# TGoldC/Motion-Planning-for-Autonomous-Driving-with-MPC

Hardware: AMD Instinct MI355X
Metric: MPC steps/sec (N=30, nx=6 nu=2) at batch=4096 (higher is better)
Workload: dtype f64; 1 GPU; N=30 nx=6 nu=2 bicycle lane-following, batch=4096/GPU, tol 1e-8; mode=converged, gpu=AMD Radeon Graphics

## Files before the change

### motion-planning-for-autonomous-driving-with-mpc_amd/csrc/mpc_host_common.h

```cpp
#pragma once
#include <cmath>
#include <cstddef>
#include <cstdint>
#include <cstdio>
#include <string>
#include <vector>

#include "../../include/mpcgpu.h"
#include "mpc_stage_math.h"

namespace mpc {

constexpr double BOUND_RELAX = 1e-8;

struct HostProblem {
    mpc_problem_desc desc{};
    std::vector<double> LB, UB;
    int has_fl = 0, has_fu = 0, has_ol = 0, has_ou = 0;
    double fl = 0, fu = 0, ol = 0, ou = 0;
    double ol_raw = 0;
    double fl_raw = 0;
    int fric_literal = 0;
    int n_mult = 0, n_z = 0;
    uint32_t lo_mask = 0, hi_mask = 0, dense_mask = 0xFFFFu;
    bool bounds_set = false;
    int NZ() const { return desc.nx + 2; }
    size_t n_w() const { return (size_t)2 * desc.N + (size_t)desc.nx * (desc.N + 1); }
    size_t n_g() const { return (size_t)1 + (size_t)desc.nx * (desc.N + 1) + (size_t)9 * (desc.N + 1); }
};

inline void apply_fric_literal(HostProblem& hp, int literal) {
    hp.fric_literal = literal ? 1 : 0;
    if (hp.bounds_set) hp.has_fl = std::isfinite(hp.fl_raw) && (hp.fl_raw > 0.0 || hp.fric_literal);
}
inline double relax_lo(double lo) { return std::isfinite(lo) ? lo - BOUND_RELAX * std::fmax(1.0, std::fabs(lo)) : -INFINITY; }
inline double relax_hi(double hi) { return std::isfinite(hi) ? hi + BOUND_RELAX * std::fmax(1.0, std::fabs(hi)) : INFINITY; }

inline int validate_desc(const mpc_problem_desc& d, std::string& err) {
    char buf[256];
    if (d.N < 1 || d.N > 127) { snprintf(buf, sizeof buf, "N=%d outside [1,127]", d.N); err = buf; return MPC_ERR_INVALID; }
    if (d.nx != 5 && d.nx != 6) { snprintf(buf, sizeof buf, "nx=%d (supported: 5, 6)", d.nx); err = buf; return MPC_ERR_INVALID; }
    if (d.nu != 2) { err = "nu must be 2"; return MPC_ERR_INVALID; }
    if (d.formulation != MPC_FORM_CASADI_EULER) { err = "unsupported formulation"; return MPC_ERR_INVALID; }
    if (!(d.dt > 0) || !(d.wheelbase > 0) || !(d.friction_div != 0) || !(d.tol > 0)) { err = "dt, wheelbase, tol must be > 0"; return MPC_ERR_INVALID; }
    if (d.obst_mult < 1 || d.max_iter < 1 || d.fixed_iters < 0) { err = "obst_mult>=1, max_iter>=1, fixed_iters>=0 required"; return MPC_ERR_INVALID; }
    if (d.max_iter > 1024 || d.fixed_iters > 1024) { err = "max_iter / fixed_iters above 1024 (the convergence-poll table)"; return MPC_ERR_INVALID; }
    return MPC_OK;
}

inline void default_bounds(const mpc_problem_desc& d, std::vector<double>& lbx, std::vector<double>& ubx,
                           std::vector<double>& lbg, std::vector<double>& ubg) {
    const int N = d.N, nx = d.nx;
    lbx.clear(); ubx.clear(); lbg.clear(); ubg.clear();
    for (int k = 0; k < N; ++k) { lbx.push_back(-0.4); ubx.push_back(0.4); lbx.push_back(-INFINITY); ubx.push_back(11.5); }
    for (int k = 0; k <= N; ++k) {
        const double lo[6] = {-INFINITY, -INFINITY, -1.066, 0.0, -INFINITY, -INFINITY};
        const double hi[6] = {INFINITY, INFINITY, 1.066, 50.8, INFINITY, INFINITY};
        for (int i = 0; i < nx; ++i) { lbx.push_back(lo[i]); ubx.push_back(hi[i]); }
    }
    lbg.push_back(0.0); ubg.push_back(11.5);
    for (int i = 0; i < nx * (N + 1); ++i) { lbg.push_back(0.0); ubg.push_back(0.0); }
    for (int i = 0; i < 9 * (N + 1); ++i) { lbg.push_back(1.2000000000000002); ubg.push_back(INFINITY); }
}

inline int set_bound_rows(HostProblem& hp, const double* lbx, const double* ubx, const double* lbg, const double* ubg, std::string& err) {
    const mpc_problem_desc& d = hp.desc;
    const int N = d.N, nx = d.nx, NZ = nx + 2;
    std::vector<double> dlbx, dubx, dlbg, dubg;
    if (!lbx && !ubx && !lbg && !ubg) {
        default_bounds(d, dlbx, dubx, dlbg, dubg);
        lbx = dlbx.data(); ubx = dubx.data(); lbg = dlbg.data(); ubg = dubg.data();
    } else if (!lbx || !ubx || !lbg || !ubg) {
        err = "lbx, ubx, lbg, ubg must be all given or all NULL";
        return MPC_ERR_INVALID;
    }
    char buf[256];
    hp.LB.assign((size_t)(N + 1) * NZ, -INFINITY);
    hp.UB.assign((size_t)(N + 1) * NZ, INFINITY);
    int nb = 0;
    for (int k = 0; k <= N; ++k)
        for (int i = 0; i < NZ; ++i) {
            if (i < 2 && k == N) continue;
            const size_t src = (i < 2) ? (size_t)2 * k + i : (size_t)2 * N + (size_t)nx * k + (i - 2);
            const double lo = lbx[src], hi = ubx[src];
            if (std::isnan(lo) || std::isnan(hi) || lo > hi) { snprintf(buf, sizeof buf, "lbx/ubx[%zu]: invalid pair", src); err = buf; return MPC_ERR_BOUNDS; }
            if (lo == hi) { snprintf(buf, sizeof buf, "lbx == ubx at %zu: fixed variables are not supported", src); err = buf; return MPC_ERR_BOUNDS; }
            hp.LB[(size_t)k * NZ + i] = relax_lo(lo);
            hp.UB[(size_t)k * NZ + i] = relax_hi(hi);
            if (!(k == 0 && i == 1)) nb += (int)std::isfinite(lo) + (int)std::isfinite(hi);
        }
    const double flo = lbg[0], fhi = ubg[0];
    if (std::isnan(flo) || std::isnan(fhi) || !(flo < fhi)) { err = "friction row needs lbg[0] < ubg[0]"; return MPC_ERR_BOUNDS; }
    for (int i = 0; i < nx * (N + 1); ++i)
        if (!(lbg[1 + i] == 0.0 && ubg[1 + i] == 0.0)) { snprintf(buf, sizeof buf, "g row %d must be an equality with lbg = ubg = 0", 1 + i); err = buf; return MPC_ERR_BOUNDS; }
    const size_t o0 = (size_t)1 + (size_t)nx * (N + 1);
    const double olo = lbg[o0], ohi = ubg[o0];
    for (int i = 0; i < 9 * (N + 1); ++i)
        if (!(lbg[o0 + i] == olo && ubg[o0 + i] == ohi)) { err = "obstacle rows must share one [lbg, ubg] pair"; return MPC_ERR_BOUNDS; }
    if (std::isnan(olo) || std::isnan(ohi) || !(olo < ohi)) { err = "obstacle rows need lbg < ubg"; return MPC_ERR_BOUNDS; }
    hp.fl_raw = flo;
    hp.has_fl = std::isfinite(flo) && (flo > 0.0 || hp.fric_literal);
    hp.has_fu = std::isfinite(fhi);
    hp.fl = relax_lo(flo); hp.fu = relax_hi(fhi);
    hp.has_ol = std::isfinite(olo); hp.has_ou = std::isfinite(ohi);
    hp.ol = relax_lo(olo); hp.ou = relax_hi(ohi);
    hp.ol_raw = olo;
    const int m = d.obst_mult;
    hp.n_mult = nx * (N + 1) + 3 * m * (N + 1);
    hp.n_z = nb + 3 * m * (N + 1) * (hp.has_ol + hp.has_ou);
    hp.bounds_set = true;
    return MPC_OK;
}
inline int set_bounds(HostProblem& hp, const double* lbx, const double* ubx, const double* lbg, const double* ubg, std::string& err) {
    const int rc = set_bound_rows(hp, lbx, ubx, lbg, ubg, err);
    hp.lo_mask = hp.hi_mask = 0;
    hp.dense_mask = 0xFFFFu;
    for (size_t q = 0; q < hp.LB.size(); ++q) {
        const int i = (int)(q % (size_t)hp.NZ()), k = (int)(q / (size_t)hp.NZ());
        if (hp.LB[q] > -1e300) hp.lo_mask |= 1u << i;
        if (hp.UB[q] < 1e300) hp.hi_mask |= 1u << i;
        if (!(i < 2 && k == hp.desc.N)) {
            if (!(hp.LB[q] > -1e300)) hp.dense_mask &= ~(1u << i);
            if (!(hp.UB[q] < 1e300)) hp.dense_mask &= ~(0x100u << i);
        }
    }
    return rc;
}

struct WsLayout {
    size_t Z, ZL, ZU, SO, NUO, ZLO, ZUO, LAM, REF, DZ, PK, KK, BLK, ROLL, SC, FILT, OBST;
    size_t MZ, MZL, MZU, MSO, MNUO, MZLO, MZUO, MLAM, MREF;
    size_t MBLK, MPK, MDZ;
    size_t rows, irows;
    size_t tile_elems, itile_elems, ntiles;
    size_t total, itotal;
    size_t elem(size_t row0, size_t row, size_t b) const { return (b >> 6) * tile_elems + mpc_prow((uint32_t)(row0 + row)) + (b & 63) * 2; }
    size_t ielem(size_t row, size_t b) const { return (b >> 6) * itile_elems + mpc_prow((uint32_t)row) + (b & 63) * 2; }
};

inline WsLayout ws_layout(int N, int nx, size_t Bp, bool mailbox = true) {
    const size_t NS = (size_t)nx * (nx + 1) / 2, S = N + 1;
    auto ev = [](size_t r) { return (r + 1) & ~(size_t)1; };
    const size_t NZ = ev(nx + 2), XS = ev(nx), NBLK = ev((nx + 5) + 10 + 2 * nx), NPK = ev(NS + nx), NKK = 2 * nx + 2;
    WsLayout w{};
    size_t off = 0;
    auto take = [&](size_t rows) { const size_t o = off; off += ev(rows); return o; };
    w.Z = take(S * NZ); w.ZL = take(S * NZ); w.ZU = take(S * NZ);
    w.SO = take(S * 4); w.NUO = take(S * 4); w.ZLO = take(S * 4); w.ZUO = take(S * 4);
    w.LAM = take(S * XS); w.REF = take(S * XS); w.DZ = take(S * NZ);
    w.PK = take(S * NPK); w.KK = take((size_t)N * NKK); w.BLK = take(S * NBLK); w.ROLL = take(S * XS);
    w.SC = take(SC_COUNT); w.FILT = take(2 * FILTER_MAX); w.OBST = take(6);
    w.rows = off;
    w.irows = ev(IS_COUNT);
    w.tile_elems = w.rows * 64;
    w.itile_elems = w.irows * 64;
    w.ntiles = Bp / 64;
    w.total = w.ntiles * w.tile_elems;
    const size_t mb = mailbox ? Bp * S : 0;
    w.MBLK = w.total; w.total += mb * NBLK;
    w.MPK = w.total; w.total += mb * NPK;
    w.MDZ = w.total; w.total += mb * NZ;
    w.MZ = w.total; w.total += mb * NZ;
    w.MZL = w.total; w.total += mb * NZ;
    w.MZU = w.total; w.total += mb * NZ;
    w.MSO = w.total; w.total += mb * 4;
    w.MNUO = w.total; w.total += mb * 4;
    w.MZLO = w.total; w.total += mb * 4;
    w.MZUO = w.total; w.total += mb * 4;
    w.MLAM = w.total; w.total += mb * XS;
    w.MREF = w.total; w.total += mb * XS;
    w.itotal = w.ntiles * w.itile_elems;
    return w;
}

inline int pick_bx(int N, int max_threads) {
    int bx = 64;
    while (bx > 4 && bx * (N + 1) > max_threads) bx >>= 1;
    return bx;
}

inline void fill_params(Params& P, const HostProblem& hp, int B, size_t Bp, int bx, double* base, int32_t* ibase,
                        const double* dLB, const double* dUB, bool mailbox = true) {
    const mpc_problem_desc& d = hp.desc;
    const WsLayout w = ws_layout(d.N, d.nx, Bp, mailbox);
    P.B = B; P.Bp = (int32_t)Bp; P.N = d.N; P.nx = d.nx; P.bx = bx;
    P.obst_mult = d.obst_mult; P.max_iter = d.max_iter; P.fixed_iters = d.fixed_iters;
    P.has_fl = hp.has_fl; P.has_fu = hp.has_fu; P.has_ol = hp.has_ol; P.has_ou = hp.has_ou; P.per_inst_obst = 0;
    P.dt = d.dt; P.wheelbase = d.wheelbase; P.friction_div = d.friction_div; P.ego_offset = d.ego_offset; P.tol = d.tol;
    for (int i = 0; i < 6; ++i) P.Q[i] = (i < d.nx) ? d.Q[i] : 0.0;
    P.R[0] = d.R[0]; P.R[1] = d.R[1];
    for (int i = 0; i < 6; ++i) P.obst[i] = d.obstacle[i];
    P.fl = hp.fl; P.fu = hp.fu; P.ol = hp.ol; P.ou = hp.ou;
    P.inv_S = (uint32_t)((0x100000000ull + (uint64_t)d.N) / (uint64_t)(d.N + 1));
    P.run_counter = nullptr;
    P.dec_s = 0;
    P.tile_mask = nullptr;
    P.lo_mask = hp.lo_mask; P.hi_mask = hp.hi_mask; P.dense_mask = hp.dense_mask;
    P.dec_s = (d.nx == 6 && d.Q[5] == 0.0 && !((P.lo_mask | P.hi_mask) & (1u << 7))) ? 1 : 0;
// ... 34 lines not shown
```

### motion-planning-for-autonomous-driving-with-mpc_amd/csrc/mpc_solve_plan.h

```cpp
#pragma once
#include <algorithm>
#include <cctype>
#include <cstdlib>
#include <cstring>
#include <string>

#include "mpc_host_common.h"

namespace mpc {

struct Knobs {
    int pipeline, hybrid, hybrid_bx, hybrid_live, pipe_help, pipe_test_abort, pipe_xcd_mask;
    int rescue, rescue_wg, rescue_alone, loop_async, sync_spin, max_batch, friction_lb, bound_mask, big_wg, groups, poison;
    int timing;
    Knobs();
};
enum class KnobParse {
    ON,
    INT,
    FLAG,
    MASK,
    FRIC,
};
struct KnobDef { const char* name; int Knobs::*field; int dflt; KnobParse parse; };
// ... 43 lines not shown
        for (const char* c = e.name; *c; ++c) env += (char)toupper(*c);
        const char* v = getenv(env.c_str());
        if (v) (void)set_knob(k, e.name, v);
    }
}

constexpr int TIMING_STAGE = 1,
              TIMING_PIPE = 2,
              TIMING_WG = 4,
              TIMING_START = 8,
              TIMING_WG_TRACE = 16;

constexpr int STAGE_MAX_THREADS = 512;
constexpr int MAX_GROUPS = 4;
constexpr int MAX_POLL_IT = 1024;
constexpr size_t LDS_MAX = 160 * 1024 - 1024;

#ifndef MPC_STAGE_STASH
#define MPC_STAGE_STASH 1
#endif
template <int NX> struct Stash {
    static constexpr int rows(bool has_ou) { return 4 * (NX + 2) + 2 * 3 + (has_ou ? 2 * 3 : 0) + 3 + 2 * NX; }
};

constexpr uint32_t REF_BOUND_VM = 0x33u;
constexpr uint32_t REF_DENSE_LO = 0x31u, REF_DENSE_HI = 0x33u;

constexpr int RIC_DEPTH = 4;
constexpr int RIC_DEPTH_F = 10;

constexpr uint32_t PIPE_X_STRIDE = 64;
enum PipeXcdWord : uint32_t { PX_ARRIVE = 0, PX_HEAD = 16, PX_TAIL = 32, PX_FINISHED = 48, PX_HO_TICKET = 56 };
constexpr uint32_t PIPE_ABORT = 8 * PIPE_X_STRIDE;
constexpr uint32_t HO_BUCKETS = 4;
enum PipeHeadWord : uint32_t {
    PH_ABORT = 0, PH_ROUNDS = 1,
    PH_STAT64 = 2,
    PH_STAGE_WORKERS = 12, PH_RIC_WORKERS = 13, PH_FAIL = 14,
    PH_WG = 16,
    PH_HELPED = 21, PH_FIN_TICKET = 22,
    PH_HO = 24,
    PH_DETAIL = 28,
    PH_WORDS = 32 };
enum PipeStat64 : uint32_t { P64_RIC_WAIT, P64_STAGE_WAIT, P64_STAGE_BUSY, P64_ITEMS };
enum WgStatWord : uint32_t { WGS_ROUNDS_MAX, WGS_ROUNDS, WGS_SWEEPS, WGS_INST_ROUNDS, WGS_RESCUED, WGS_WORDS };
constexpr uint32_t PIPE_STATS = PIPE_ABORT + PH_STAT64, PIPE_WG = PIPE_ABORT + PH_WG, PIPE_HO = PIPE_ABORT + PH_HO, PIPE_HDR = PIPE_ABORT + PH_WORDS;
struct CtlField { uint32_t at, words, align; };
template <size_t N> constexpr bool ctl_fields_ok(const CtlField (&f)[N], uint32_t size) {
    for (size_t i = 0; i < N; ++i) {
        if (f[i].at % f[i].align || f[i].at + f[i].words > size) return false;
        for (size_t j = 0; j < i; ++j) if (f[i].at < f[j].at + f[j].words && f[j].at < f[i].at + f[i].words) return false;
    }
    return true;
}
constexpr CtlField PIPE_HEAD_FIELDS[] = {{PH_ABORT, 1, 1}, {PH_ROUNDS, 1, 1}, {PH_STAT64, 8, 2}, {PH_STAGE_WORKERS, 1, 1}, {PH_RIC_WORKERS, 1, 1}, {PH_FAIL, 1, 1},
                                         {PH_WG, WGS_WORDS, 1}, {PH_HELPED, 1, 1}, {PH_FIN_TICKET, 1, 1}, {PH_HO, HO_BUCKETS, 1}, {PH_DETAIL, 4, 1}};
constexpr CtlField PIPE_XCD_FIELDS[] = {{PX_ARRIVE, 1, 1}, {PX_HEAD, 1, 1}, {PX_TAIL, 1, 1}, {PX_FINISHED, 1, 1}, {PX_HO_TICKET, 1, 1}};
static_assert(ctl_fields_ok(PIPE_HEAD_FIELDS, PH_WORDS) && PIPE_ABORT % 2 == 0 && PH_HO + HO_BUCKETS <= PH_DETAIL, "the head's fields are disjoint, inside it, the uint64 ones 8-byte aligned; the hand-over counters end in front of the abort details");
static_assert(ctl_fields_ok(PIPE_XCD_FIELDS, PIPE_X_STRIDE), "the fields of an XCD record are disjoint and inside it");
constexpr uint32_t pipe_slots_off(uint32_t ntiles) { return (PIPE_HDR + ntiles + 1u) & ~1u; }
constexpr size_t pipe_ctl_words(uint32_t ntiles, uint32_t cap) { return (size_t)pipe_slots_off(ntiles) + (size_t)16 * cap; }
constexpr int PIPE_MAX_TILES = 256;

constexpr size_t prestart_doubles(int NX, int S, int bx) { return (size_t)4 * S * (NX + 2) + (size_t)(3 * NX + 2) * S * bx + (size_t)4 * bx; }
template <int NX>
struct WgLds {
    static constexpr int PAD = Rec<NX>::SIZE > 64 ? Rec<NX>::SIZE : 64;
    static constexpr size_t doubles(int S, int bxw) { return (size_t)PAD + (size_t)Rec<NX>::SIZE * S * bxw + (size_t)2 * S * (NX + 2) + (size_t)16 * bxw + (size_t)64 * NX + (size_t)WgScl::SIZE * bxw; }
};

struct PlanState {
    int n_cu = 256;
    uint32_t xcd_mask = 0xFFu;
    bool ws_mailbox = false;
    bool pipe_disabled = false;
    bool resc_hint = false;
    int32_t B = 0;
    bool per_inst_obst = false;
    bool trace = false;
    bool in_rescue = false;
    bool async_loop = false;
};
struct SolvePlan {
    bool small_wg;
    int S, bx, threads, nblk, ntiles, G, stash_rows;
    size_t lds_bytes, lds_init, ric_lds;
    bool masked;
    int cap, chunk;
    bool polled;
    bool fused;
    size_t lds_pre, lds_start;
    bool res_path, pipe_path;
    int hyb_bx;
    bool resc_alone, hyb_ok;
    int hand;
    bool wg_resc;
    size_t wg_lds;
    int wg_grid;
    uint32_t xcd_mask;
    int n_xcd, tiles_x, cu_x, n_ric;
    uint32_t pipe_cap;
    bool pipe_help;
    int mbw_live;
    bool stage_timing, start_timing, wg_timing, wg_trace, pipe_timing, poison;
    size_t max_rows;
    bool mailbox;
    bool rescue;
    bool loop_async;
};

template <int NX>
SolvePlan plan_solve_nx(const HostProblem& hp, const Knobs& kn, const PlanState& st) {
    const mpc_problem_desc& d = hp.desc;
    const int B = st.B;
    SolvePlan pl{};
    const size_t Bp = ((size_t)B + 63) / 64 * 64;
    const int S = d.N + 1;
    pl.S = S;
    pl.ntiles = (int)(Bp / 64);
    const int ntiles = pl.ntiles;
    pl.small_wg = 4 * S <= 256 && !kn.big_wg;
    pl.bx = pick_bx(d.N, pl.small_wg ? 256 : STAGE_MAX_THREADS);
    const int bx = pl.bx;
    pl.threads = ((S * bx + 63) / 64) * 64;
    pl.nblk = (B + bx - 1) / bx;
    pl.stage_timing = (kn.timing & TIMING_STAGE) != 0;
    const int nw = pl.threads / 64;
    pl.stash_rows = pl.small_wg && MPC_STAGE_STASH ? std::max(Stash<NX>::rows(hp.has_ou != 0), 2 * NX) : 2 * NX;
    pl.lds_bytes = ((size_t)nw * 10 * bx + (size_t)2 * S * (NX + 2) + (size_t)pl.stash_rows * pl.threads) * sizeof(double);
    pl.lds_init = ((size_t)nw * 10 * bx + (size_t)2 * S * (NX + 2) + (size_t)2 * NX * pl.threads) * sizeof(double);
    pl.ric_lds = std::max(RIC_DEPTH * (size_t)((MPC_EV(Dim<NX>::NBLK) * 512 + 1023) / 1024) * 1024,
                          RIC_DEPTH_F * (size_t)((Dim<NX>::NKK * 512 + 1023) / 1024 + 6) * 1024) + 64;
    pl.G = 1;
    if (!st.trace && !pl.stage_timing && kn.groups > 0) pl.G = std::min(std::max(std::min(kn.groups, ntiles / 4), 1), MAX_GROUPS);
    const int G = pl.G;
    const bool ref_vm_ok = ((hp.lo_mask | hp.hi_mask) & ~REF_BOUND_VM) == 0u;
    pl.masked = kn.bound_mask != 0 && ref_vm_ok && (hp.dense_mask & REF_DENSE_LO) == REF_DENSE_LO && ((hp.dense_mask >> 8) & REF_DENSE_HI) == REF_DENSE_HI &&
                hp.has_ol && !hp.has_ou && d.obst_mult == 3 && !st.per_inst_obst;
    pl.cap = d.fixed_iters > 0 ? d.fixed_iters : d.max_iter;
    pl.chunk = d.fixed_iters > 0 ? pl.cap : 4;
    pl.polled = d.fixed_iters <= 0 && !st.trace;
    const int n_w = 2 * d.N + NX * (d.N + 1);
    pl.lds_pre = prestart_doubles(NX, S, bx) * sizeof(double);
    const size_t lds_in = (size_t)bx * (2 * n_w - 2 * d.N) * sizeof(double);
    const size_t lds_red = (size_t)(pl.threads / 64) * 10 * bx * sizeof(double);
    pl.fused = lds_red + pl.lds_pre + 16 + lds_in <= 78 * 1024 && d.N >= 1 && pl.small_wg;
    pl.lds_start = std::max(lds_red + pl.lds_pre + 16 + lds_in, pl.lds_init);

    auto wg_lds = [&](int bxw) {
        const size_t pre = prestart_doubles(NX, S, bxw) * sizeof(double);
        const size_t init = ((size_t)10 * bxw + (size_t)2 * S * (NX + 2) + (size_t)2 * NX * 64) * sizeof(double);
        return std::max(WgLds<NX>::doubles(S, bxw) * sizeof(double), bxw == 1 ? std::max(pre, init) : (size_t)0);
    };
    pl.rescue = kn.rescue && d.fixed_iters <= 0 && !st.trace && hp.has_ol && hp.ol_raw > 0.0;
    const bool resc_cond = pl.rescue && (kn.rescue_wg >= 2 || kn.rescue_alone || (kn.rescue_wg == 1 && st.resc_hint)) && !st.in_rescue;
    int hyb_bx = ((kn.hybrid_bx == 2 || (kn.hybrid_bx == 0 && B > 4 * st.n_cu)) && S * 2 <= 64) ? 2 : 1;
    if (kn.hybrid_bx == 0 && resc_cond && hyb_bx == 2 && (size_t)ntiles * 64 * 8 <= (size_t)4 * st.n_cu * 18) hyb_bx = 1;
    pl.resc_alone = kn.rescue_alone && kn.hybrid_bx == 0 && kn.hybrid_live < 0 && resc_cond && ntiles <= 128;
    if (pl.resc_alone || st.in_rescue) hyb_bx = 1;
    pl.hyb_bx = hyb_bx;
    pl.wg_resc = resc_cond && hyb_bx == 1;
    pl.wg_lds = wg_lds(hyb_bx);
    pl.mailbox = pl.small_wg && S <= 64 && kn.hybrid && d.fixed_iters <= 0 && kn.pipeline && !st.pipe_disabled;
    pl.hyb_ok = kn.hybrid && st.ws_mailbox && d.fixed_iters <= 0 && kn.pipeline && !st.pipe_disabled && G == 1 && pl.small_wg && S <= 64 &&
                pl.wg_lds <= LDS_MAX / 4 && !st.trace && !pl.stage_timing;
    int hand = 0;
    if (pl.hyb_ok) {
        const int base = std::min(64, 4 * st.n_cu * hyb_bx / std::max(1, ntiles));
        hand = base >= 64 ? base : std::max(base, std::min(50, base < 32 ? 7 * base / 4 : 3 * base / 2));
        if (hyb_bx == 1 && base < 64 && hand < 40) hand = 40;
        if ((size_t)ntiles * 64 * 8 <= (size_t)4 * st.n_cu * hyb_bx * (hyb_bx == 2 ? 9 : 18)) hand = 64;
        if (pl.resc_alone) hand = 64;
        if (kn.hybrid_live >= 0) hand = std::min(64, kn.hybrid_live);
    }
    pl.hand = hand;
    pl.res_path = pl.hyb_ok && (hand >= 64 || st.in_rescue);
    pl.xcd_mask = st.xcd_mask;
    if (kn.pipe_xcd_mask) {
        const uint32_t m = (uint32_t)kn.pipe_xcd_mask & st.xcd_mask;
        if (m) pl.xcd_mask = m;
    }
    pl.n_xcd = __builtin_popcount(pl.xcd_mask);
    pl.tiles_x = (ntiles + pl.n_xcd - 1) / pl.n_xcd;
    pl.cu_x = std::max(2, st.n_cu / pl.n_xcd);
    const int tiles_x = pl.tiles_x, cu_x = pl.cu_x;
    const int n_ric_base = std::max(1, cu_x / 4);
    const bool ric_per_tile = tiles_x > n_ric_base && tiles_x <= 3 * cu_x / 8 && (64 / bx) * tiles_x <= 5 * (cu_x - tiles_x) && S >= 24;
    pl.n_ric = std::min(ric_per_tile ? tiles_x : n_ric_base, tiles_x);
    const bool eligible = G == 1 && !st.trace && !pl.stage_timing && pl.small_wg && pl.threads >= 192 && pl.threads <= 256 &&
                          ntiles <= (d.fixed_iters > 0 ? 64 : PIPE_MAX_TILES) && (tiles_x + pl.n_ric - 1) / pl.n_ric <= 32 &&
                          std::max(pl.lds_bytes, pl.ric_lds) <= LDS_MAX;
    pl.pipe_path = !pl.res_path && eligible && !st.pipe_disabled && kn.pipeline;
    pl.pipe_cap = 1;
    while (pl.pipe_path && pl.pipe_cap < 2u * (64u / (uint32_t)bx) * (uint32_t)tiles_x) pl.pipe_cap <<= 1;
    pl.pipe_help = pl.pipe_path && pl.masked && (kn.pipe_help < 0 ? (64 / bx) * tiles_x > 3 * (cu_x - pl.n_ric) : kn.pipe_help != 0);
    pl.mbw_live = pl.pipe_path && hand > 0 ? std::min(63, hand + 16) : 0;
    pl.wg_grid = pl.res_path ? (B + hyb_bx - 1) / hyb_bx
               : pl.pipe_path && hand > 0 ? std::min((B + hyb_bx - 1) / hyb_bx, std::max(4 * st.n_cu, (int)((size_t)hand * ntiles + hyb_bx - 1) / hyb_bx)) : 0;
    pl.start_timing = (kn.timing & TIMING_START) && !st.async_loop && G == 1;
    pl.wg_timing = (kn.timing & TIMING_WG) && !st.async_loop;
    pl.wg_trace = (kn.timing & TIMING_WG_TRACE) && !st.async_loop && !st.in_rescue;
    pl.pipe_timing = (kn.timing & TIMING_PIPE) != 0;
    pl.poison = kn.poison && !st.in_rescue;

    const WsLayout w1 = ws_layout(d.N, NX, 64, pl.mailbox);
    pl.max_rows = (((size_t)1 << 32) - 1) / (w1.total * sizeof(double)) * 64;
    const bool pipe_shape = pl.small_wg && kn.pipeline && !st.pipe_disabled && kn.groups <= 0 && !pl.stage_timing && d.fixed_iters <= 0 &&
                            pl.threads >= 192 && pl.threads <= 256;
    if (pipe_shape) pl.max_rows = std::min(pl.max_rows, (size_t)PIPE_MAX_TILES * 64);
    if (kn.max_batch > 0) pl.max_rows = std::min(pl.max_rows, (size_t)(kn.max_batch + 63) / 64 * 64);
    pl.loop_async = d.fixed_iters <= 0 && kn.pipeline && !st.pipe_disabled && kn.loop_async && (size_t)B <= pl.max_rows;
    return pl;
}
inline SolvePlan plan_solve(const HostProblem& hp, const Knobs& kn, const PlanState& st) {
    return hp.desc.nx == 5 ? plan_solve_nx<5>(hp, kn, st) : plan_solve_nx<6>(hp, kn, st);
}

struct SolveIo {
    int32_t B = 0;
    const double *x0 = nullptr, *p = nullptr, *obst = nullptr;
    double *x_out = nullptr, *kkt = nullptr;
    int32_t *status = nullptr, *iters = nullptr;
    double *lam_g = nullptr, *lam_x = nullptr;
    double* snap = nullptr;
    size_t n_w = 0, n_g = 0, snap_len = 0;
    struct Trace { double* out = nullptr; int32_t rows = 0; int32_t* n_it = nullptr; } trace;
    SolveIo rows(size_t off, int32_t n) const {
        SolveIo r = *this;
        r.B = n; r.trace = Trace{};
        skip(r.x0, off * n_w); skip(r.p, off * n_w); skip(r.obst, off * 6);
        skip(r.x_out, off * n_w); skip(r.status, off * 1); skip(r.iters, off * 1); skip(r.kkt, off * 1);
        skip(r.lam_g, off * n_g); skip(r.lam_x, off * n_w); skip(r.snap, off * snap_len);
        return r;
    }
    template <class T> static void skip(T*& q, size_t elems) { if (q) q += elems; }
};

}
```

### motion-planning-for-autonomous-driving-with-mpc_amd/csrc/mpcgpu.hip

```cpp
#include <hip/hip_runtime.h>
#include <type_traits>

#include <algorithm>
#include <cctype>
#include <cstdio>
#include <cstdlib>
#include <cstring>
#include <new>
#include <string>
#include <vector>

#include "mpc_host_common.h"
#include "mpc_solve_plan.h"
#include "mpc_stamps.h"
#include "mpc_closed_loop.h"
#include "mpc_forces_qp.h"
#include "mpc_riccati_mfma.h"
#include "mpc_sens.h"

using namespace mpc;

namespace {

__device__ __forceinline__ void lds_barrier() {
// ... 1245 lines not shown
    int frow = 1;
    if (valid && c.k == 0) {
        if (WS) frow = prestart_a0<NX>(P, c.b, a0lb, a0ub);
        else frow = prestart_a0_of<NX>(P, src.ref0(bl, 2), src.ref0(bl, 3), a0lb, a0ub);
        A0[bl] = a0lb;
        A0[bx + bl] = a0ub;
    }
    __syncthreads();
    MPC_STAMP(P.DBG, blockIdx.x, PP_BOUNDS, threadIdx.x == 0);
    const double dt = P.dt;
#define PP_AT(arr, i, k) (arr)[((i) * S + (k)) * bx + bl]
    if (valid) {
        const int k = c.k;
        double g[NX];
#pragma unroll
        for (int i = 0; i < NX; ++i) g[i] = fmin(fmax(WS ? (double)MPC_K(P.Z, NZ, 0, 2 + i) : src.z(bl, k, 2 + i), PLt[k * NZ + 2 + i]), PHt[k * NZ + 2 + i]);
        if (k == 0) {
#pragma unroll
            for (int i = 0; i < NX; ++i) {
                const double r0 = WS ? (double)MPC_K(P.REF, NX, 0, i) : src.ref0(bl, i);
                const double x0 = fmin(fmax(r0, PLt[2 + i]), PHt[2 + i]);
                PP_AT(XR, i, 0) = x0;
                PP_AT(DR, i, 0) = fabs(x0 - r0);
                PP_AT(DG, i, 0) = fabs(g[i] - r0);
            }
        }
        if (k < N) {
            double u[2], f[NX], sp, cp, td;
            u[0] = fmin(fmax(WS ? (double)MPC_K(P.Z, NZ, 0, 0) : src.z(bl, k, 0), PLt[k * NZ]), PHt[k * NZ]);
            {
                const double u1 = WS ? (double)MPC_K(P.Z, NZ, 0, 1) : src.z(bl, k, 1);
                u[1] = (k == 0) ? push_in(u1, A0[bl], A0[bx + bl]) : fmin(fmax(u1, PLt[k * NZ + 1]), PHt[k * NZ + 1]);
            }
            PP_AT(IN, 0, k) = u[0];
            PP_AT(IN, 1, k) = u[1];
            ode_eval<NX>(P, g, u, f, sp, cp, td);
#pragma unroll
            for (int i = 0; i < NX; ++i) {
                const double raw = f[i] * dt + g[i];
                const double gn = fmin(fmax(WS ? (double)MPC_K(P.Z, NZ, 1, 2 + i) : src.z(bl, k + 1, 2 + i), PLt[(k + 1) * NZ + 2 + i]), PHt[(k + 1) * NZ + 2 + i]);
                PP_AT(DG, i, k + 1) = fabs(gn - raw);
            }
        }
    }
    __syncthreads();
    MPC_STAMP(P.DBG, blockIdx.x, PP_DEFECTS, threadIdx.x == 0);
    auto defect_sum = [&](const double* D, double th, const int ka, const int kb) {
        for (int k0 = ka; k0 < kb; k0 += 4) {
            double v[4][NX];
#pragma unroll
            for (int j = 0; j < 4; ++j) {
                const int k = (k0 + j < kb) ? k0 + j : kb - 1;
#pragma unroll
                for (int i = 0; i < NX; ++i) v[j][i] = PP_AT(D, i, k);
            }
#pragma unroll
            for (int j = 0; j < 4; ++j) {
                if (k0 + j < kb) {
#pragma unroll
                    for (int i = 0; i < NX; ++i) th += v[j][i];
                }
            }
        }
        return th;
    };
    const int kdg = (64 / bx <= N) ? 64 / bx : 1;
    const bool sums_dg = valid && c.k == kdg;
    double th_g = 0.0;
    int dg_part = 0;
    if (valid && c.k == 0) A0[3 * bx + bl] = 0.0;
    bool clipped = false;
    auto scan = [&](int s0, int s1, int nwhich) {
        if (sums_dg) {
            th_g = defect_sum(DG, th_g, dg_part * S / 3, (dg_part + 1) * S / 3);
            if (++dg_part == 3) A0[2 * bx + bl] = th_g;
        }
        if (valid && c.k < nwhich) {
            const int si = (c.k == 0) ? s0 : s1;
            const double* in = IN + c.k * SB;
            double x = PP_AT(XR, si, 0);
            int k0 = 0;
            for (; k0 + 8 <= N; k0 += 8) {
                double inc[8], lo[8], hi[8];
#pragma unroll
                for (int j = 0; j < 8; ++j) { const int k = k0 + j; inc[j] = in[k * bx + bl]; lo[j] = PLt[(k + 1) * NZ + 2 + si]; hi[j] = PHt[(k + 1) * NZ + 2 + si]; }
#pragma unroll
                for (int j = 0; j < 8; ++j) {
                    x = fmin(fmax(__builtin_fma(inc[j], dt, x), lo[j]), hi[j]);
                    PP_AT(XR, si, k0 + j + 1) = x;
                }
            }
            if (k0 < N) {
                double inc[8], lo[8], hi[8];
#pragma unroll
                for (int j = 0; j < 8; ++j) { const int k = (k0 + j < N) ? k0 + j : N - 1; inc[j] = in[k * bx + bl]; lo[j] = PLt[(k + 1) * NZ + 2 + si]; hi[j] = PHt[(k + 1) * NZ + 2 + si]; }
#pragma unroll
                for (int j = 0; j < 8; ++j) {
                    if (k0 + j < N) {
                        x = fmin(fmax(__builtin_fma(inc[j], dt, x), lo[j]), hi[j]);
                        PP_AT(XR, si, k0 + j + 1) = x;
                    }
                }
            }
        }
        __syncthreads();
        if (valid && c.k < N) {
            for (int w = 0; w < nwhich; ++w) {
                const int si = w ? s1 : s0;
                const double raw = __builtin_fma(PP_AT(IN + w * SB, 0, c.k), dt, PP_AT(XR, si, c.k));
                const double dr = fabs(PP_AT(XR, si, c.k + 1) - raw);
                PP_AT(DR, si, c.k + 1) = dr;
                clipped = clipped || dr != 0.0;
            }
        }
    };
    scan(2, 3, 2);
    MPC_STAMP(P.DBG, blockIdx.x, PP_SCAN1, threadIdx.x == 0);
    if (valid && c.k < N) {
        const double dl = PP_AT(XR, 2, c.k), v = PP_AT(XR, 3, c.k);
        PP_AT(IN, 0, c.k) = v / P.wheelbase * mpc_tan(dl);
        PP_AT(IN, 1, c.k) = v;
    }
    __syncthreads();
    scan(4, 5, NX == 6 ? 2 : 1);
    MPC_STAMP(P.DBG, blockIdx.x, PP_SCAN2, threadIdx.x == 0);
    if (valid && c.k < N) {
        double sp, cp;
        mpc_sincos(PP_AT(XR, 4, c.k), sp, cp);
        const double v = PP_AT(XR, 3, c.k);
        PP_AT(IN, 0, c.k) = v * cp;
        PP_AT(IN, 1, c.k) = v * sp;
    }
    __syncthreads();
    scan(0, 1, 2);
    MPC_STAMP(P.DBG, blockIdx.x, PP_SCAN3, threadIdx.x == 0);
    if (valid) {
#pragma unroll
        for (int i = 0; i < NX; ++i) MPC_K(P.ROLL, NX, 0, i) = PP_AT(XR, i, c.k);
        if (clipped) A0[3 * bx + bl] = 1.0;
    }
    __syncthreads();
    MPC_STAMP(P.DBG, blockIdx.x, PP_SUMS, threadIdx.x == 0);
    if (valid && c.k == 0) {
        double th = 0.0;
        if (A0[3 * bx + bl] != 0.0) th = defect_sum(DR, 0.0, 0, S);
        else {
#pragma unroll
            for (int i = 0; i < NX; ++i) th += PP_AT(DR, i, 0);
        }
        prestart_decide<NX>(P, c.b, frow, a0lb, a0ub, A0[2 * bx + bl], th);
    }
#undef PP_AT
}
template <int NX>
__global__ void __launch_bounds__(1024) k_prestart_par(const Params Pk) {
    const PRef P(Pk);
    extern __shared__ __attribute__((aligned(16))) double sm[];
    prestart_par_block<NX>(P, (blockIdx.x + (uint32_t)P.tile0 * (64u / (uint32_t)P.bx)) * (uint32_t)P.bx, sm);
}
#ifndef MPC_KSTART_OCC
#define MPC_KSTART_OCC 2
#endif
template <int NX>
__global__ void __launch_bounds__(256, MPC_KSTART_OCC) k_start(const Params Pk, const int n_mult, const int n_z, const int stash_rows, uint32_t* zero_p, const uint32_t zero_n) {
    const PRef P(Pk);
    extern __shared__ __attribute__((aligned(16))) double lds[];
    if (zero_p != nullptr && blockIdx.x == 0)
        for (uint32_t q = threadIdx.x; q < zero_n; q += blockDim.x) zero_p[q] = 0u;
    uint32_t blk = blockIdx.x;
    if ((gridDim.x & 7u) == 0u) blk = (blk & 7u) * (gridDim.x >> 3) + (blk >> 3);
    const uint32_t b0 = (blk + (uint32_t)P.tile0 * (64u / (uint32_t)P.bx)) * (uint32_t)P.bx;
    MPC_STAMP(P.DBG, blockIdx.x, KS_BEGIN, threadIdx.x == 0);
    {
        constexpr int NZ = NX + 2;
        const int N = P.N, nw = 2 * N + NX * (N + 1), bx = P.bx, t = threadIdx.x;
        const size_t pre_doubles = prestart_doubles(NX, N + 1, bx);
        double* const pre = lds + (blockDim.x >> 6) * 10 * bx;
        double* rx = pre + ((pre_doubles + 1) & ~(size_t)1);
        double* rp = rx + bx * nw;
        const int nrow = ((int)b0 + bx <= P.B) ? bx : (P.B > (int)b0 ? P.B - (int)b0 : 0);
        const int npx = nw - 2 * N;
        batched_fill<8>(nrow * nw, t, (int)blockDim.x, [&](int q) { return MPC_GP(P.x0, (size_t)b0 * nw + q); }, [&](int q, double v) { rx[q] = v; });
        for (int r0 = 0; r0 < nrow; r0 += 8) {
            for (int c0 = 0; c0 < npx; c0 += (int)blockDim.x) {
                const int col = c0 + t;
                double v[8];
#pragma unroll
                for (int r = 0; r < 8; ++r) v[r] = (r0 + r < nrow && col < npx) ? (double)MPC_GP(P.p, ((size_t)b0 + r0 + r) * nw + 2 * N + col) : 0.0;
#pragma unroll
                for (int r = 0; r < 8; ++r) if (r0 + r < nrow && col < npx) rp[(r0 + r) * npx + col] = v[r];
            }
        }
        __syncthreads();
        MPC_STAMP(P.DBG, blockIdx.x, KS_ROWS, threadIdx.x == 0);
        struct { int b, k; } c;
        c.k = t / bx;
        const int bl = t & (bx - 1);
        c.b = (int)b0 + bl;
        if (c.k <= N && c.b < P.B) {
            double z[NZ], r[NX];
            const double* xr = rx + bl * nw;
            z[0] = (c.k < N) ? xr[2 * c.k] : 0.0;
            z[1] = (c.k < N) ? xr[2 * c.k + 1] : 0.0;
#pragma unroll
            for (int i = 0; i < NX; ++i) { z[2 + i] = xr[2 * N + NX * c.k + i]; r[i] = rp[bl * npx + NX * c.k + i]; }
            ws_store_rows<NZ>(MPC_ROWS(MPC_K(P.Z, NZ, 0, e)), z);
            ws_store_rows<NX>(MPC_ROWS(MPC_K(P.REF, NX, 0, e)), r);
        }
        struct FromLds {
            const double *rx, *rp;
            int nw, npx, N;
            __device__ __forceinline__ double z(int bl, int k, int i) const { return i < 2 ? (k < N ? rx[bl * nw + 2 * k + i] : 0.0) : rx[bl * nw + 2 * N + NX * k + (i - 2)]; }
            __device__ __forceinline__ double ref0(int bl, int i) const { return rp[bl * npx + i]; }
        } src{rx, rp, nw, npx, N};
        MPC_STAMP(P.DBG, blockIdx.x, KS_STORED, threadIdx.x == 0);
        prestart_par_block<NX, FromLds>(P, b0, pre, src);
    }
    MPC_STAMP(P.DBG, blockIdx.x, KS_SAFE, threadIdx.x == 0);
    asm volatile("s_waitcnt vmcnt(0)" ::: "memory");
    __syncthreads();
    __builtin_amdgcn_fence(__ATOMIC_ACQ_REL, "workgroup");
    asm volatile("s_waitcnt vmcnt(0)" ::: "memory");
    MPC_STAMP(P.DBG, blockIdx.x, KS_FENCED, threadIdx.x == 0);
    stage_block<NX, true, 256>(P, n_mult, n_z, stash_rows, b0, ~0ull, lds, true, nullptr, true);
}


template <int NX>
__device__ __forceinline__ uint32_t zrow_of_col(int col, int N) {
    constexpr int NZ = NX + 2;
    if (col < 2 * N) return (uint32_t)(col >> 1) * MPC_EV(NZ) + (uint32_t)(col & 1);
    const int cx = col - 2 * N;
    return (uint32_t)(cx / NX) * MPC_EV(NZ) + 2u + (uint32_t)(cx % NX);
}

template <int NX>
__global__ void __launch_bounds__(256) k_ingest(const Params Pk) {
    const PRef P(Pk);
    __shared__ double tile[64][65];
    const int N = P.N, nw = 2 * N + NX * (N + 1);
    const uint32_t tl = blockIdx.x + (uint32_t)P.tile0, t0 = tl * 64u;
    const int lane = threadIdx.x & 63, w = threadIdx.x >> 6;
    double* Zt = P.Z + (size_t)tl * P.tile_elems;
    double* Rt = P.REF + (size_t)tl * P.tile_elems;
    const int nc0 = (nw + 63) / 64;
    const int pass = (int)blockIdx.y < nc0 ? 0 : 1;
    const int c0 = pass == 0 ? (int)blockIdx.y * 64 : 2 * N + ((int)blockIdx.y - nc0) * 64;
    const double* src = pass == 0 ? P.x0 : P.p;
    for (int r = w; r < 64; r += 4) {
        const int col = c0 + lane;
        const uint32_t b = t0 + (uint32_t)r;
        tile[r][lane] = (col < nw && b < (uint32_t)P.B) ? src[(size_t)b * nw + col] : 0.0;
    }
    __syncthreads();
    for (int cc = w; cc < 64; cc += 4) {
        const int col = c0 + cc;
        if (col < nw) {
            if (pass == 0) Zt[mpc_prow(zrow_of_col<NX>(col, N)) + 2u * lane] = tile[lane][cc];
            else Rt[mpc_prow((uint32_t)((col - 2 * N) / NX) * MPC_EV(NX) + (uint32_t)((col - 2 * N) % NX)) + 2u * lane] = tile[lane][cc];
        }
    }
    constexpr int NZ = NX + 2;
    if (blockIdx.y == 0 && threadIdx.x < 128) Zt[mpc_prow((uint32_t)N * MPC_EV(NZ) + (threadIdx.x >> 6)) + 2u * lane] = 0.0;
}

template <int NX>
__global__ void __launch_bounds__(256) k_egest(const Params Pk, const uint32_t* skip_if, uint32_t* fail_count, uint32_t* zero_p, const uint32_t zero_n) {
    const PRef P(Pk);
    __shared__ double tile[64][65];
    if (zero_p != nullptr && blockIdx.x == 0 && blockIdx.y == 0)
        for (uint32_t q = threadIdx.x; q < zero_n; q += 256u) zero_p[q] = 0u;
    if (skip_if != nullptr && *skip_if != 0u) return;
    const int N = P.N, nw = 2 * N + NX * (N + 1);
    const uint32_t tl = blockIdx.x + (uint32_t)P.tile0, t0 = tl * 64u;
    const int lane = threadIdx.x & 63, w = threadIdx.x >> 6;
    const double* Zt = P.Z + (size_t)tl * P.tile_elems;
    const int c0 = (int)blockIdx.y * 64;
    for (int cc = w; cc < 64; cc += 4) {
        const int col = c0 + cc;
        tile[lane][cc] = (col < nw) ? Zt[mpc_prow(zrow_of_col<NX>(col, N)) + 2u * lane] : 0.0;
    }
    __syncthreads();
    for (int r = w; r < 64; r += 4) {
        const int col = c0 + lane;
        const uint32_t b = t0 + (uint32_t)r;
        if (col < nw && b < (uint32_t)P.B) P.x_out[(size_t)b * nw + col] = tile[r][lane];
    }
    if (blockIdx.y != 0) return;
    if (threadIdx.x < 64) {
        const uint32_t b = t0 + (uint32_t)lane;
        int st = 1;
        if (b < (uint32_t)P.B) {
            st = P.ISC[tl * P.itile_elems + mpc_prow((uint32_t)IS_STATUS) + 2u * lane];
            if (st == ST_RUNNING) st = 0;
            if (P.status_out) P.status_out[b] = st;
            if (P.iters_out) P.iters_out[b] = P.ISC[tl * P.itile_elems + mpc_prow((uint32_t)IS_ITERS) + 2u * lane];
            if (P.kkt_out) P.kkt_out[b] = P.SC[(size_t)tl * P.tile_elems + mpc_prow((uint32_t)SC_E0) + 2u * lane];
        }
        const int nbad = __popcll(__ballot((st == 0 || st == -7) ? 1 : 0));
        if (fail_count != nullptr && lane == 0 && nbad) atomicAdd(fail_count, (uint32_t)nbad);
    }
}

__global__ void k_count_running(const int32_t* iws, uint32_t itile_elems, int b0, int B, int32_t* counter) {
    const int b = b0 + (int)(blockIdx.x * blockDim.x + threadIdx.x);
    const int run = (b < B && iws[((uint32_t)b >> 6) * itile_elems + mpc_prow((uint32_t)IS_STATUS) + 2u * ((uint32_t)b & 63u)] == ST_RUNNING) ? 1 : 0;
    const unsigned long long m = __ballot(run);
    if ((threadIdx.x & 63) == 0 && m) atomicAdd(counter, (int)__popcll(m));
}

__global__ void k_transpose_obst(const double* obst , double* OBST , int B, uint32_t tile_elems) {
    const int b = blockIdx.x * blockDim.x + threadIdx.x;
    if (b >= B) return;
#pragma unroll
    for (int i = 0; i < 6; ++i) OBST[((uint32_t)b >> 6) * tile_elems + mpc_prow((uint32_t)i) + 2u * ((uint32_t)b & 63u)] = obst[(size_t)b * 6 + i];
}

__global__ void k_gather_trace(const double* SC , uint32_t tile_elems, int B, double* out) {
    const int b = blockIdx.x * blockDim.x + threadIdx.x;
    if (b >= B) return;
    const int rows[8] = {SC_MU, SC_THETA, SC_PHI, SC_ALPHA, SC_ADU, SC_DELTA, SC_E0, SC_NTRIAL};
#pragma unroll
    for (int q = 0; q < 8; ++q) out[(size_t)q * B + b] = SC[((uint32_t)b >> 6) * tile_elems + mpc_prow((uint32_t)rows[q]) + 2u * ((uint32_t)b & 63u)];
}

__device__ __forceinline__ double sqrt_cr(double x) {
    const double r = sqrt(x);
    if (!(r > 0.0) || !isfinite(r)) return r;
    return fma(fma(-r, r, x), 0.5 / r, r);
}

__global__ void __launch_bounds__(256) k_metrics(int L, int Lo, const double* traj, const double* ref_path, const double* origin_path,
                                                 const double* obst, double ego_offset, double r_sum, int all_pairs, double* deviation,
                                                 double* rmsd, double* clearance) {
#pragma clang fp contract(off)
    __shared__ double red[256];
    const int b = blockIdx.x, t = threadIdx.x;
    const double* x = traj + (size_t)b * L * 5;
    if (deviation != nullptr && origin_path != nullptr) {
        const double* op = origin_path + (size_t)b * Lo * 2;
        for (int i = t; i < L; i += 256) {
            const double px = x[i * 5], py = x[i * 5 + 1];
            double best = INFINITY;
            int arg = 0;
            for (int q = 0; q < Lo; ++q) {
                const double dx = op[2 * q] - px, dy = op[2 * q + 1] - py;
                const double sq = dx * dx + dy * dy;
                if (sq < best) { best = sq; arg = q; }
            }
            const double ex = op[2 * arg] - px, ey = op[2 * arg + 1] - py;
            deviation[(size_t)b * L + i] = sqrt_cr(ex * ex + ey * ey);
        }
    }
    if (rmsd != nullptr && ref_path != nullptr && t == 0) {
        const double* rp = ref_path + (size_t)b * L * 2;
        double sx = 0.0, sy = 0.0;
        for (int i = 0; i < L; ++i) {
            const double dx = rp[2 * i] - x[i * 5], dy = rp[2 * i + 1] - x[i * 5 + 1];
            sx = sx + dx * dx;
            sy = sy + dy * dy;
        }
        rmsd[(size_t)b * 2] = sqrt_cr(sx / (double)(L - 1));
        rmsd[(size_t)b * 2 + 1] = sqrt_cr(sy / (double)(L - 1));
    }
    if (clearance != nullptr) {
        double best = INFINITY;
        for (int i = t; i < L; i += 256) {
            const double sx = x[i * 5], sy = x[i * 5 + 1], psi = x[i * 5 + 4];
            double sn, cs;
// ... 1950 lines not shown
```

Measured before the change: 5.327 million MPC steps/s.

## Pipeline prestart rollout chains across waves in fused k_start

Adds a prestart variant that splits the sequential state rollout into chunks of 8 steps and staggers them across wave roles (position chain, heading/velocity inputs, trig inputs, defect sum), so the dependent scans overlap in a software pipeline instead of running one after another. The fused k_start kernel now calls this variant in place of the previous parallel prestart. It also lets max_iter be 0 and disables the rescue, hybrid, pipeline and async-loop paths when the iteration cap is zero. This adds more barriers per stage and role-dependent branching, and the LDS layout gains extra PL/PH tables.

Measured after the change: 5.240 million MPC steps/s. 0.984x the previous value.

```diff
diff --git a/motion-planning-for-autonomous-driving-with-mpc_amd/csrc/mpc_host_common.h b/motion-planning-for-autonomous-driving-with-mpc_amd/csrc/mpc_host_common.h
--- a/motion-planning-for-autonomous-driving-with-mpc_amd/csrc/mpc_host_common.h
+++ b/motion-planning-for-autonomous-driving-with-mpc_amd/csrc/mpc_host_common.h
@@ -43,7 +43,7 @@
     if (d.nu != 2) { err = "nu must be 2"; return MPC_ERR_INVALID; }
     if (d.formulation != MPC_FORM_CASADI_EULER) { err = "unsupported formulation"; return MPC_ERR_INVALID; }
     if (!(d.dt > 0) || !(d.wheelbase > 0) || !(d.friction_div != 0) || !(d.tol > 0)) { err = "dt, wheelbase, tol must be > 0"; return MPC_ERR_INVALID; }
-    if (d.obst_mult < 1 || d.max_iter < 1 || d.fixed_iters < 0) { err = "obst_mult>=1, max_iter>=1, fixed_iters>=0 required"; return MPC_ERR_INVALID; }
+    if (d.obst_mult < 1 || d.max_iter < 0 || d.fixed_iters < 0) { err = "obst_mult>=1, max_iter>=0, fixed_iters>=0 required"; return MPC_ERR_INVALID; }
     if (d.max_iter > 1024 || d.fixed_iters > 1024) { err = "max_iter / fixed_iters above 1024 (the convergence-poll table)"; return MPC_ERR_INVALID; }
     return MPC_OK;
 }
diff --git a/motion-planning-for-autonomous-driving-with-mpc_amd/csrc/mpc_solve_plan.h b/motion-planning-for-autonomous-driving-with-mpc_amd/csrc/mpc_solve_plan.h
--- a/motion-planning-for-autonomous-driving-with-mpc_amd/csrc/mpc_solve_plan.h
+++ b/motion-planning-for-autonomous-driving-with-mpc_amd/csrc/mpc_solve_plan.h
@@ -219,7 +219,7 @@
         const size_t init = ((size_t)10 * bxw + (size_t)2 * S * (NX + 2) + (size_t)2 * NX * 64) * sizeof(double);
         return std::max(WgLds<NX>::doubles(S, bxw) * sizeof(double), bxw == 1 ? std::max(pre, init) : (size_t)0);
     };
-    pl.rescue = kn.rescue && d.fixed_iters <= 0 && !st.trace && hp.has_ol && hp.ol_raw > 0.0;
+    pl.rescue = kn.rescue && d.fixed_iters <= 0 && !st.trace && hp.has_ol && hp.ol_raw > 0.0 && pl.cap > 0;
     const bool resc_cond = pl.rescue && (kn.rescue_wg >= 2 || kn.rescue_alone || (kn.rescue_wg == 1 && st.resc_hint)) && !st.in_rescue;
     int hyb_bx = ((kn.hybrid_bx == 2 || (kn.hybrid_bx == 0 && B > 4 * st.n_cu)) && S * 2 <= 64) ? 2 : 1;
     if (kn.hybrid_bx == 0 && resc_cond && hyb_bx == 2 && (size_t)ntiles * 64 * 8 <= (size_t)4 * st.n_cu * 18) hyb_bx = 1;
@@ -230,7 +230,7 @@
     pl.wg_lds = wg_lds(hyb_bx);
     pl.mailbox = pl.small_wg && S <= 64 && kn.hybrid && d.fixed_iters <= 0 && kn.pipeline && !st.pipe_disabled;
     pl.hyb_ok = kn.hybrid && st.ws_mailbox && d.fixed_iters <= 0 && kn.pipeline && !st.pipe_disabled && G == 1 && pl.small_wg && S <= 64 &&
-                pl.wg_lds <= LDS_MAX / 4 && !st.trace && !pl.stage_timing;
+                pl.wg_lds <= LDS_MAX / 4 && !st.trace && !pl.stage_timing && pl.cap > 0;
     int hand = 0;
     if (pl.hyb_ok) {
         const int base = std::min(64, 4 * st.n_cu * hyb_bx / std::max(1, ntiles));
@@ -254,7 +254,7 @@
     const int n_ric_base = std::max(1, cu_x / 4);
     const bool ric_per_tile = tiles_x > n_ric_base && tiles_x <= 3 * cu_x / 8 && (64 / bx) * tiles_x <= 5 * (cu_x - tiles_x) && S >= 24;
     pl.n_ric = std::min(ric_per_tile ? tiles_x : n_ric_base, tiles_x);
-    const bool eligible = G == 1 && !st.trace && !pl.stage_timing && pl.small_wg && pl.threads >= 192 && pl.threads <= 256 &&
+    const bool eligible = G == 1 && !st.trace && !pl.stage_timing && pl.small_wg && pl.threads >= 192 && pl.threads <= 256 && pl.cap > 0 &&
                           ntiles <= (d.fixed_iters > 0 ? 64 : PIPE_MAX_TILES) && (tiles_x + pl.n_ric - 1) / pl.n_ric <= 32 &&
                           std::max(pl.lds_bytes, pl.ric_lds) <= LDS_MAX;
     pl.pipe_path = !pl.res_path && eligible && !st.pipe_disabled && kn.pipeline;
@@ -276,7 +276,7 @@
                             pl.threads >= 192 && pl.threads <= 256;
     if (pipe_shape) pl.max_rows = std::min(pl.max_rows, (size_t)PIPE_MAX_TILES * 64);
     if (kn.max_batch > 0) pl.max_rows = std::min(pl.max_rows, (size_t)(kn.max_batch + 63) / 64 * 64);
-    pl.loop_async = d.fixed_iters <= 0 && kn.pipeline && !st.pipe_disabled && kn.loop_async && (size_t)B <= pl.max_rows;
+    pl.loop_async = d.fixed_iters <= 0 && kn.pipeline && !st.pipe_disabled && kn.loop_async && (size_t)B <= pl.max_rows && pl.cap > 0;
     return pl;
 }
 inline SolvePlan plan_solve(const HostProblem& hp, const Knobs& kn, const PlanState& st) {
diff --git a/motion-planning-for-autonomous-driving-with-mpc_amd/csrc/mpcgpu.hip b/motion-planning-for-autonomous-driving-with-mpc_amd/csrc/mpcgpu.hip
--- a/motion-planning-for-autonomous-driving-with-mpc_amd/csrc/mpcgpu.hip
+++ b/motion-planning-for-autonomous-driving-with-mpc_amd/csrc/mpcgpu.hip
@@ -1421,6 +1421,170 @@
     }
 #undef PP_AT
 }
+template <int NX, class Src>
+__device__ __forceinline__ void prestart_pipe_block(const PRef& P, const uint32_t b0, double* sm, const Src src) {
+    constexpr int NZ = NX + 2, CH = 8;
+    const int N = P.N, S = N + 1, bx = P.bx, t = threadIdx.x, bl = t & (bx - 1);
+    const int nb = S * NZ, SB = S * bx;
+    double* LBt = sm;
+    double* UBt = LBt + nb;
+    double* XR = UBt + nb;
+    double* DR = XR + NX * SB;
+    double* DG = DR + NX * SB;
+    double* IN = DG + NX * SB;
+    double* A0 = IN + 2 * SB;
+    double* PLt = A0 + 4 * bx;
+    double* PHt = PLt + nb;
+    struct { int b, k; } c;
+    c.k = t / bx;
+    c.b = (int)b0 + bl;
+    const bool inst = c.b < P.B, valid = c.k <= N && inst;
+    for (int q0 = 0; q0 < nb; q0 += 2 * (int)blockDim.x) {
+        double lo[2], hi[2];
+#pragma unroll
+        for (int j = 0; j < 2; ++j) { const int q = q0 + j * (int)blockDim.x + t; lo[j] = q < nb ? (double)MPC_GP(P.LB, q) : 0.0; hi[j] = q < nb ? (double)MPC_GP(P.UB, q) : 0.0; }
+#pragma unroll
+        for (int j = 0; j < 2; ++j) {
+            const int q = q0 + j * (int)blockDim.x + t;
+            if (q < nb) { double L, H; push_limits(lo[j], hi[j], L, H); LBt[q] = lo[j]; UBt[q] = hi[j]; PLt[q] = L; PHt[q] = H; }
+        }
+    }
+    double a0lb = 0.0, a0ub = 0.0;
+    int frow = 1;
+    if (valid && c.k == 0) {
+        frow = prestart_a0_of<NX>(P, src.ref0(bl, 2), src.ref0(bl, 3), a0lb, a0ub);
+        A0[bl] = a0lb;
+        A0[bx + bl] = a0ub;
+        A0[3 * bx + bl] = 0.0;
+    }
+    __syncthreads();
+    MPC_STAMP(P.DBG, blockIdx.x, PP_BOUNDS, threadIdx.x == 0);
+    const double dt = P.dt;
+#define PP_AT(arr, i, k) (arr)[((i) * S + (k)) * bx + bl]
+    if (valid) {
+        const int k = c.k;
+        double g[NX];
+#pragma unroll
+        for (int i = 0; i < NX; ++i) g[i] = fmin(fmax(src.z(bl, k, 2 + i), PLt[k * NZ + 2 + i]), PHt[k * NZ + 2 + i]);
+        if (k == 0) {
+#pragma unroll
+            for (int i = 0; i < NX; ++i) {
+                const double r0 = src.ref0(bl, i);
+                const double x0 = fmin(fmax(r0, PLt[2 + i]), PHt[2 + i]);
+                PP_AT(XR, i, 0) = x0;
+                PP_AT(DR, i, 0) = fabs(x0 - r0);
+                PP_AT(DG, i, 0) = fabs(g[i] - r0);
+            }
+        }
+        if (k < N) {
+            double u[2], f[NX], sp, cp, td;
+            u[0] = fmin(fmax(src.z(bl, k, 0), PLt[k * NZ]), PHt[k * NZ]);
+            {
+                const double u1 = src.z(bl, k, 1);
+                u[1] = (k == 0) ? push_in(u1, A0[bl], A0[bx + bl]) : fmin(fmax(u1, PLt[k * NZ + 1]), PHt[k * NZ + 1]);
+            }
+            PP_AT(IN, 0, k) = u[0];
+            PP_AT(IN, 1, k) = u[1];
+            ode_eval<NX>(P, g, u, f, sp, cp, td);
+#pragma unroll
+            for (int i = 0; i < NX; ++i) {
+                const double raw = f[i] * dt + g[i];
+                const double gn = fmin(fmax(src.z(bl, k + 1, 2 + i), PLt[(k + 1) * NZ + 2 + i]), PHt[(k + 1) * NZ + 2 + i]);
+                PP_AT(DG, i, k + 1) = fabs(gn - raw);
+            }
+        }
+    }
+    __syncthreads();
+    MPC_STAMP(P.DBG, blockIdx.x, PP_DEFECTS, threadIdx.x == 0);
+    const int wave = lds_uniform(t >> 6), lane = t & 63, nwv = (int)(blockDim.x >> 6), lbx = 31 - __clz(bx);
+    const int nch = (N + CH - 1) / CH, nst = nch + 2;
+    bool clipped = false;
+    auto chain = [&](const int which, const int si, const int k0) {
+        const double* in = IN + which * SB;
+        double x = PP_AT(XR, si, k0);
+        double inc[CH], lo[CH], hi[CH];
+#pragma unroll
+        for (int j = 0; j < CH; ++j) { const int k = (k0 + j < N) ? k0 + j : N - 1; inc[j] = in[k * bx + bl]; lo[j] = PLt[(k + 1) * NZ + 2 + si]; hi[j] = PHt[(k + 1) * NZ + 2 + si]; }
+#pragma unroll
+        for (int j = 0; j < CH; ++j) {
+            if (k0 + j < N) {
+                const double raw = __builtin_fma(inc[j], dt, x);
+                x = fmin(fmax(raw, lo[j]), hi[j]);
+                const double dr = fabs(x - raw);
+                PP_AT(XR, si, k0 + j + 1) = x;
+                PP_AT(DR, si, k0 + j + 1) = dr;
+                clipped = clipped || dr != 0.0;
+            }
+        }
+    };
+    double th_g = 0.0;
+    for (int s = 0; s < nst; ++s) {
+        for (int role = wave; role < 4; role += nwv) {
+            const int k0 = (s - role) * CH;
+            if (role == 3) {
+                if (inst && lane < bx) {
+                    const int kb = (s + 1) * S / nst;
+                    for (int k = s * S / nst; k < kb; ++k) {
+                        double v[NX];
+#pragma unroll
+                        for (int i = 0; i < NX; ++i) v[i] = PP_AT(DG, i, k);
+#pragma unroll
+                        for (int i = 0; i < NX; ++i) th_g += v[i];
+                    }
+                    if (s == nst - 1) A0[2 * bx + bl] = th_g;
+                }
+            } else if (k0 >= 0 && k0 < N) {
+                if (role != 0) {
+                    for (int e0 = 0; e0 < CH * bx; e0 += 64) {
+                        const int k = k0 + ((e0 + lane) >> lbx);
+                        if (inst && k < k0 + CH && k < N) {
+                            const double v = PP_AT(XR, 3, k);
+                            if (role == 1) {
+                                PP_AT(IN, 0, k) = v / P.wheelbase * mpc_tan(PP_AT(XR, 2, k));
+                                PP_AT(IN, 1, k) = v;
+                            } else {
+                                double sp, cp;
+                                mpc_sincos(PP_AT(XR, 4, k), sp, cp);
+                                PP_AT(IN, 0, k) = v * cp;
+                                PP_AT(IN, 1, k) = v * sp;
+                            }
+                        }
+                    }
+                    asm volatile("s_waitcnt lgkmcnt(0)" ::: "memory");
+                }
+                const int s0 = role == 0 ? 2 : role == 1 ? 4 : 0, nwhich = (role == 1 && NX == 5) ? 1 : 2;
+                for (int q0 = 0; q0 < nwhich * bx; q0 += 64) {
+                    const int which = (q0 + lane) >> lbx;
+                    if (inst && which < nwhich) chain(which, s0 + which, k0);
+                }
+            }
+            MPC_STAMP(P.DBG, blockIdx.x, role == 0 ? PP_SCAN1 : PP_SCAN2, lane == 0 && role < 2 && s == nch - 1 + role);
+        }
+        lds_barrier();
+    }
+    MPC_STAMP(P.DBG, blockIdx.x, PP_SCAN3, threadIdx.x == 0);
+    if (valid) {
+#pragma unroll
+        for (int i = 0; i < NX; ++i) MPC_K(P.ROLL, NX, 0, i) = PP_AT(XR, i, c.k);
+    }
+    if (clipped) A0[3 * bx + bl] = 1.0;
+    __syncthreads();
+    MPC_STAMP(P.DBG, blockIdx.x, PP_SUMS, threadIdx.x == 0);
+    if (valid && c.k == 0) {
+        double th = 0.0;
+        if (A0[3 * bx + bl] != 0.0) {
+            for (int k = 0; k < S; ++k) {
+#pragma unroll
+                for (int i = 0; i < NX; ++i) th += PP_AT(DR, i, k);
+            }
+        } else {
+#pragma unroll
+            for (int i = 0; i < NX; ++i) th += PP_AT(DR, i, 0);
+        }
+        prestart_decide<NX>(P, c.b, frow, a0lb, a0ub, A0[2 * bx + bl], th);
+    }
+#undef PP_AT
+}
 template <int NX>
 __global__ void __launch_bounds__(1024) k_prestart_par(const Params Pk) {
     const PRef P(Pk);
@@ -1483,7 +1647,7 @@
             __device__ __forceinline__ double ref0(int bl, int i) const { return rp[bl * npx + i]; }
         } src{rx, rp, nw, npx, N};
         MPC_STAMP(P.DBG, blockIdx.x, KS_STORED, threadIdx.x == 0);
-        prestart_par_block<NX, FromLds>(P, b0, pre, src);
+        prestart_pipe_block<NX, FromLds>(P, b0, pre, src);
     }
     MPC_STAMP(P.DBG, blockIdx.x, KS_SAFE, threadIdx.x == 0);
     asm volatile("s_waitcnt vmcnt(0)" ::: "memory");
```
